# jianzhnie/RLZero

Measured on AMD Instinct MI355X. Metric: mcts_sims_per_sec, higher is better.
Workload: dtype f32 net (hi + lo f16 operand pairs on the f16 MFMA pipe, f32 accumulation) / f64 tree

## Files before the change

### include/rlzero_hip.h

```cpp
#ifndef RLZERO_HIP_H
#define RLZERO_HIP_H

#include <stdint.h>

#ifdef __cplusplus
extern "C" {
#endif

#define RZ_ABI_VERSION 27
#define RZ_MAX_BOARD_SIZE 16
#define RZ_BOARD_WORDS 4
#define RZ_MAX_IN_FLIGHT 16

enum {
    RZ_OK = 0,
    RZ_ERR_ARG = -1,
    RZ_ERR_HIP = -2,
    RZ_ERR_OOM = -3,
    RZ_ERR_OVERFLOW = -4,
    RZ_ERR_ILLEGAL = -5,
    RZ_ERR_INTERNAL = -6
};

enum {
    RZ_GAME_GOMOKU = 0,
    RZ_GAME_CONNECT4 = 1
};

enum {
    RZ_SCORE_UCT_REF = 0,
    RZ_SCORE_PUCT = 1
};

enum { RZ_EVAL_V0 = 0, RZ_EVAL_VLIN = 1 };

enum {
    RZ_FLAG_ARENA_FULL = 1,
    RZ_FLAG_BLOCKS_FULL = 2,
    RZ_FLAG_ILLEGAL_MOVE = 4,
    RZ_FLAG_LOGTAB = 8,
    RZ_FLAG_INTERNAL = 16,
    RZ_FLAG_REUSE_DROPPED = 32
// ... 82 lines not shown
    const float *act_bias;
    const float *val_scale;
    const float *val_bias;
    int64_t raw_part_stride;
    int64_t hid_part_stride;
    int32_t ld;
    int32_t n_parts;
} rz_raw_heads;

int rz_expand_backup_raw(rz_engine *e, const rz_raw_heads *heads, void *stream);
int rz_tree_step_raw(rz_engine *e, const rz_raw_heads *heads, float *d_obs, void *stream);

typedef struct rz_value_head {
    const float *valfeat;
    const float *w1t;
    const float *b1;
    const float *w2;
    const float *b2;
    int32_t ld;
    int32_t groups;
} rz_value_head;
typedef struct rz_deferred_logits {
    const float *raw;
    int32_t ld;
    int32_t rows_per_slot;
} rz_deferred_logits;
int rz_deferred_reserve(rz_engine *e, int32_t slots);
int rz_trace_attach(rz_engine *e, void *d_trace);
int rz_device_view(rz_engine *e, void *out, int64_t out_bytes);
int rz_deferred_slots(rz_engine *e, const int32_t **d_slot_of_game);
int rz_expand_backup_deferred(rz_engine *e, const rz_value_head *head, void *stream);
int rz_tree_step_deferred(rz_engine *e, const rz_value_head *head, void *stream);
int rz_deferred_flush(rz_engine *e, const rz_deferred_logits *logits, int32_t n_slots, void *stream);

int rz_root_visits(rz_engine *e, int32_t *d_visits, void *stream);
int rz_root_wsum(rz_engine *e, double *d_w, void *stream);
int rz_root_priors(rz_engine *e, float *d_p, void *stream);
int rz_root_stats(rz_engine *e, int32_t *d_n, double *d_w, void *stream);
int rz_root_values(rz_engine *e, double *d_out, void *stream);

int rz_advance_roots(rz_engine *e, const int32_t *d_moves, void *stream);

int rz_step_games(rz_engine *e, const int32_t *d_moves, int32_t *d_winner, uint8_t *d_ended,
                  void *stream);

#define RZ_PLAY_RECORD_WORDS 8
enum {
    RZ_PLAY_RUNNING = 1,
    RZ_PLAY_STALLED = 2,
    RZ_PLAY_RESOLVED = 4,
    RZ_PLAY_ENDED = 8,
    RZ_PLAY_SEARCHED = 16,
    RZ_PLAY_RESIGNED = 32,
    RZ_PLAY_NO_RESIGN = 64,
    RZ_PLAY_WOULD_RESIGN = 128
};
typedef struct rz_play_config {
    uint64_t seed;
    double temperature;
    double stall_margin;
    const int64_t *d_queue_ids;
    int32_t *d_queue_ctl;
    int32_t *d_log;
    int32_t ring_steps;
    int32_t reserved;
} rz_play_config;
// ... 16 lines not shown

int rz_uct_scores(rz_engine *e, const double *d_w, const int32_t *d_n, const int32_t *d_np,
                  double c_puct, double *d_out, int64_t count, void *stream);

typedef struct rz_net rz_net;
enum {
    RZ_NET_DIRECT = 0,
    RZ_NET_WINOGRAD_F4 = 1,
    RZ_NET_SPLIT_F16 = 2
    ,
    RZ_NET_SPLIT_F16_TILES = 3
    ,
    RZ_NET_SPLIT_F16_FP8 = 4
};
int rz_net_range_info(rz_net *net, float *h_info8);
enum { RZ_NET_FLAG_F16_RANGE = 1 };
int rz_net_error_flags(rz_net *net, uint32_t *h_flags);
int rz_net_set_algo(rz_net *net, int32_t algo);
int rz_net_set_max_workgroups(rz_net *net, int32_t max_workgroups);
enum { RZ_NET_HEADS_AUTO = 0, RZ_NET_HEADS_F32 = 1, RZ_NET_HEADS_SPLIT_32 = 2, RZ_NET_HEADS_SPLIT_64 = 3, RZ_NET_HEADS_SPLIT_PARTS = 4,
       RZ_NET_HEADS_IN_TRUNK = 5    };
int rz_net_set_heads_algo(rz_net *net, int32_t heads_algo);
int rz_net_create(int32_t height, int32_t width, int32_t n_actions, int32_t device, rz_net **out);
int rz_net_destroy(rz_net *net);
int rz_net_load(rz_net *net, const float *const *h_params, int32_t n_params);
int rz_net_reserve(rz_net *net, int32_t max_boards);
int rz_net_trunk(rz_net *net, const float *d_obs, int32_t n_boards, float *d_feat, void *stream);
int rz_net_trunk_leaves(rz_net *net, const uint64_t *d_stones, const int32_t *d_to_move, const int32_t *d_last_cell,
                        int32_t n_boards, void *stream);
int rz_net_deferred_reserve(rz_net *net, int32_t max_boards, int32_t slots);
int rz_net_trunk_leaves_deferred(rz_net *net, const uint64_t *d_stones, const int32_t *d_to_move, const int32_t *d_last_cell,
                                 int32_t n_boards, const int32_t *d_slot_of_board, rz_value_head *out, void *stream);
int rz_net_deferred_gemm(rz_net *net, int32_t n_boards, int32_t n_slots, rz_deferred_logits *out, void *stream);
int rz_net_trace_attach(rz_net *net, void *d_trace);
int rz_net_delta_reserve(rz_net *net, int32_t n_games);
int rz_net_delta_invalidate(rz_net *net, void *stream);
int rz_net_delta_resident(rz_net *net, int32_t on);
int rz_net_delta_bases(rz_net *net, const uint64_t *d_root_stones, const int32_t *d_root_to_move, int32_t n_games, void *stream);
int rz_net_delta_leaves(rz_net *net, const uint64_t *d_stones, const int32_t *d_to_move, const int32_t *d_last_cell, int32_t n_boards,
                        const int32_t *d_slot_of_board, const uint8_t *d_active, float *d_feat32, int32_t without_base, rz_value_head *out,
                        void *stream);
int rz_net_delta_bases_engine(rz_net *net, rz_engine *engine, void *stream);
int rz_net_delta_step(rz_net *net, rz_engine *engine, rz_value_head *out, void *stream);
int rz_net_delta_trunk_engine(rz_net *net, rz_engine *engine, void *stream);
int rz_net_delta_stats(rz_net *net, uint32_t *h_out8, int32_t reset);
int rz_net_search_resident(rz_net *net, rz_engine *engine, int32_t n_sims, int32_t select_first, void *stream);
int rz_net_heads(rz_net *net, int32_t n_boards, float *d_logp, float *d_value, void *stream);
int rz_net_heads_gemm(rz_net *net, int32_t n_boards, rz_raw_heads *out, void *stream);
int rz_net_forward(rz_net *net, const float *d_obs, int32_t n_boards, float *d_logp,
                   float *d_value, void *stream);

typedef struct rz_muzero rz_muzero;
typedef struct rz_mz_config {
    int32_t abi_version;
    int32_t n_games;
    int32_t n_actions;
    int32_t n_sims;
    double discount;
    double pb_c_base;
    double pb_c_init;
    int32_t device;
    int32_t reserved;
} rz_mz_config;

int rz_mz_create(const rz_mz_config *cfg, rz_muzero **out);
int rz_mz_destroy(rz_muzero *e);
// ... 38 lines not shown
```

### rlzero_amd/_hip.py

```python
import ctypes
import os
from ctypes import (POINTER, Structure, c_char_p, c_double, c_int, c_int32, c_int64, c_uint32, c_uint64,
                    c_void_p)

ABI_VERSION = 27
BOARD_WORDS = 4
MAX_BOARD_SIZE = 16
MAX_IN_FLIGHT = 16

OK = 0
SCORE_UCT_REF, SCORE_PUCT = 0, 1
GAME_GOMOKU, GAME_CONNECT4 = 0, 1
NET_DIRECT, NET_WINOGRAD_F4, NET_SPLIT_F16, NET_SPLIT_F16_TILES, NET_SPLIT_F16_FP8 = 0, 1, 2, 3, 4
NET_FLAG_F16_RANGE = 1
NET_HEADS_AUTO, NET_HEADS_F32, NET_HEADS_SPLIT_32, NET_HEADS_SPLIT_64, NET_HEADS_SPLIT_PARTS, NET_HEADS_IN_TRUNK = 0, 1, 2, 3, 4, 5
EVAL_V0, EVAL_VLIN = 0, 1
FLAG_NAMES = {1: 'arena full', 2: 'block queue full', 4: 'illegal move', 8: 'ln table too short',
              16: 'internal'}
FLAG_REUSE_DROPPED = 32


class RzConfig(Structure):
    _fields_ = [('abi_version', c_int32), ('game_kind', c_int32), ('board_size', c_int32),
                ('n_in_row', c_int32), ('n_games', c_int32), ('n_playout', c_int32),
                ('score_mode', c_int32), ('add_noise', c_int32), ('c_puct', c_double),
                ('pool_factor', c_double), ('device', c_int32), ('noise_seed', c_int32),
                ('board_height', c_int32), ('board_width', c_int32),
                ('sims_in_flight', c_int32), ('in_flight_impl', c_int32)]


class RzStats(Structure):
    _fields_ = [('error_flags', c_int32), ('first_bad_game', c_int32), ('arena_slots', c_int64),
                ('prior_floats', c_int64), ('max_slots_used', c_int64), ('max_blocks_used', c_int64),
                ('device_bytes', c_int64), ('n_select_calls', c_int64), ('reuse_dropped', c_int64)]


class RzMzConfig(Structure):
    _fields_ = [('abi_version', c_int32), ('n_games', c_int32), ('n_actions', c_int32), ('n_sims', c_int32),
# ... 45 lines not shown
    'rz_last_error': (c_char_p, []),
    'rz_source_hash': (c_char_p, []),
    'rz_create': (c_int, [POINTER(RzConfig), POINTER(c_void_p)]),
    'rz_destroy': (c_int, [P]),
    'rz_geometry': (c_int, [P, POINTER(c_int32), POINTER(c_int32), POINTER(c_int32)]),
    'rz_upload_log_table': (c_int, [P, P, c_int64]),
    'rz_log_table_size': (c_int, [P, POINTER(c_int64)]),
    'rz_set_roots': (c_int, [P, P, P, P, P, c_int, P]),
    'rz_get_roots': (c_int, [P, P, P, P, P]),
    'rz_set_active': (c_int, [P, P, P]),
    'rz_set_noise_keys': (c_int, [P, P, P, P]),
    'rz_select_step': (c_int, [P, P, P]),
    'rz_set_in_flight': (c_int, [P, c_int32, c_int32]),
    'rz_leaf_buffers': (c_int, [P, POINTER(c_void_p), POINTER(c_void_p), POINTER(c_void_p)]),
    'rz_encode_leaf_obs': (c_int, [P, P, P]),
    'rz_encode_root_obs': (c_int, [P, P, P]),
    'rz_get_leaves': (c_int, [P, P, P, P, P, P]),
    'rz_eval_synthetic': (c_int, [P, c_int, P, P, P]),
    'rz_eval_rollout': (c_int, [P, c_uint64, c_uint32, c_int32, P, P]),
    'rz_expand_backup': (c_int, [P, P, P, P]),
    'rz_expand_backup_f64': (c_int, [P, P, P, P]),
    'rz_expand_backup_probs': (c_int, [P, P, P, P]),
    'rz_tree_step': (c_int, [P, P, P, P, P]),
    'rz_expand_backup_raw': (c_int, [P, POINTER(RzRawHeads), P]),
    'rz_tree_step_raw': (c_int, [P, POINTER(RzRawHeads), P, P]),
    'rz_trace_attach': (c_int, [P, P]),
    'rz_net_trace_attach': (c_int, [P, P]),
    'rz_device_view': (c_int, [P, P, c_int64]),
    'rz_deferred_reserve': (c_int, [P, c_int32]),
    'rz_deferred_slots': (c_int, [P, POINTER(c_void_p)]),
    'rz_expand_backup_deferred': (c_int, [P, POINTER(RzValueHead), P]),
    'rz_tree_step_deferred': (c_int, [P, POINTER(RzValueHead), P]),
    'rz_deferred_flush': (c_int, [P, POINTER(RzDeferredLogits), c_int32, P]),
    'rz_root_visits': (c_int, [P, P, P]),
    'rz_root_wsum': (c_int, [P, P, P]),
    'rz_root_priors': (c_int, [P, P, P]),
    'rz_root_stats': (c_int, [P, P, P, P]),
    'rz_root_values': (c_int, [P, P, P]),
    'rz_advance_roots': (c_int, [P, P, P]),
    'rz_step_games': (c_int, [P, P, P, P, P]),
    'rz_play_attach': (c_int, [P, POINTER(RzPlayConfig)]),
    'rz_play_draw': (c_int, [P, P]),
    'rz_play_apply': (c_int, [P, P]),
    'rz_play_set_resign': (c_int, [P, c_double, c_double, P]),
    'rz_play_resolve': (c_int, [P, c_int32, c_int32, P]),
    'rz_play_stop': (c_int, [P, P]),
    'rz_play_state': (c_int, [P, P, P, P, POINTER(c_int64)]),
    'rz_get_stats': (c_int, [P, POINTER(RzStats)]),
    'rz_clear_errors': (c_int, [P]),
    'rz_poll_errors': (c_int, [P, POINTER(c_int32), POINTER(c_int32), P]),
    'rz_copy_arena': (c_int, [P, c_int32, c_int64, P, P, P, P, P, P, P, P]),
    'rz_copy_priors': (c_int, [P, c_int32, c_int64, P, P]),
    'rz_uct_scores': (c_int, [P, P, P, P, c_double, P, c_int64, P]),
    'rz_net_create': (c_int, [c_int32, c_int32, c_int32, c_int32, POINTER(c_void_p)]),
    'rz_net_destroy': (c_int, [P]),
    'rz_net_set_algo': (c_int, [P, c_int32]),
    'rz_net_set_max_workgroups': (c_int, [P, c_int32]),
    'rz_net_set_heads_algo': (c_int, [P, c_int32]),
    'rz_net_error_flags': (c_int, [P, POINTER(ctypes.c_uint32)]),
    'rz_net_range_info': (c_int, [P, POINTER(ctypes.c_float)]),
    'rz_net_load': (c_int, [P, POINTER(c_void_p), c_int32]),
    'rz_net_reserve': (c_int, [P, c_int32]),
    'rz_net_trunk': (c_int, [P, P, c_int32, P, P]),
    'rz_net_trunk_leaves': (c_int, [P, P, P, P, c_int32, P]),
    'rz_net_deferred_reserve': (c_int, [P, c_int32, c_int32]),
    'rz_net_trunk_leaves_deferred': (c_int, [P, P, P, P, c_int32, P, POINTER(RzValueHead), P]),
    'rz_net_deferred_gemm': (c_int, [P, c_int32, c_int32, POINTER(RzDeferredLogits), P]),
    'rz_net_search_resident': (c_int, [P, P, c_int32, c_int32, P]),
    'rz_net_delta_reserve': (c_int, [P, c_int32]),
    'rz_net_delta_invalidate': (c_int, [P, P]),
    'rz_net_delta_resident': (c_int, [P, c_int32]),
    'rz_net_delta_bases': (c_int, [P, P, P, c_int32, P]),
    'rz_net_delta_leaves': (c_int, [P, P, P, P, c_int32, P, P, P, c_int32, POINTER(RzValueHead), P]),
    'rz_net_delta_stats': (c_int, [P, POINTER(ctypes.c_uint32), c_int32]),
    'rz_net_delta_bases_engine': (c_int, [P, P, P]),
    'rz_net_delta_step': (c_int, [P, P, POINTER(RzValueHead), P]),
    'rz_net_delta_trunk_engine': (c_int, [P, P, P]),
    'rz_net_heads': (c_int, [P, c_int32, P, P, P]),
    'rz_net_heads_gemm': (c_int, [P, c_int32, POINTER(RzRawHeads), P]),
    'rz_net_forward': (c_int, [P, P, c_int32, P, P, P]),
    'rz_mz_create': (c_int, [POINTER(RzMzConfig), POINTER(c_void_p)]),
    'rz_mz_destroy': (c_int, [P]),
    'rz_mz_upload_log_table': (c_int, [P, P, c_int64]),
    'rz_mz_init_roots': (c_int, [P, P, P, c_double, P, P]),
    'rz_mz_select': (c_int, [P, P, P, P, P, P]),
    'rz_mz_expand_backup': (c_int, [P, P, P, P, P, P]),
    'rz_mz_load_model': (c_int, [P, POINTER(c_void_p), c_int32, c_int32]),
    'rz_mz_search': (c_int, [P, P, c_int32, P, P, P, P, P, P, P]),
    'rz_mz_set_search_shape': (c_int, [P, c_int32]),
    'rz_mz_load_representation': (c_int, [P, POINTER(c_void_p), c_int32, c_int32, c_int32]),
    'rz_mz_play_cartpole': (c_int, [P, P, c_int32, c_int32, POINTER(RzMzCartPolePlay), P]),
    'rz_cartpole_step': (c_int, [P, P, P, P, c_int32, c_uint64, P, P, P, P, P]),
    'rz_mz_root_children': (c_int, [P, c_int32, P, P]),
    'rz_mz_root_stats': (c_int, [P, P, P, P, P, P]),
    'rz_mz_geometry': (c_int, [P, POINTER(c_int32), POINTER(c_int64)]),
    'rz_mz_error_flags': (c_int, [P, POINTER(c_int32)]),
}

_lib = None

# ... 39 lines not shown
```

### rlzero_amd/csrc/rz_engine.hip

```cpp

#include <hip/hip_runtime.h>

#include <cmath>
#include <cstdarg>
#include <cstdio>
#include <cstring>
#include <new>
#include <vector>

#include "rlzero_hip.h"
#include "rz_trace.h"

#pragma clang fp contract(off)

#include "rz_tree.h"

using namespace rzt;

namespace {

__global__ __launch_bounds__(kWave) void k_select(Dev E, float *obs) {
    __builtin_amdgcn_s_setprio(3);
    select_body<false>(E, obs, blockIdx.x, threadIdx.x);
}
// ... 19 lines not shown
template <int PER> constexpr int words_of_per() { return PER <= 4 ? 1 : (PER == 8 ? 2 : kWords); }
template <int PER>
__global__ __launch_bounds__(kWave * kDefWaves) void k_expand_backup_def(Dev E, ValueHead vh) {
    __shared__ float part[kDefWaves][kWave];
    __builtin_amdgcn_s_setprio(3);
    const int lane = threadIdx.x & (kWave - 1), wave = __builtin_amdgcn_readfirstlane(threadIdx.x / kWave);
    value_quarter_def<PER>(vh, blockIdx.x, lane, wave, part);
    if (wave != 0) {
        __syncthreads();
        return;
    }
    expand_backup_body<float, false, false, false, true, words_of_per<PER>()>(E, nullptr, nullptr, blockIdx.x, lane, RawHeads(), 0, vh, part);
}

template <int PER, bool TRACE>
__global__ __launch_bounds__(kWave * kDefWaves) void k_tree_step_def(Dev E, ValueHead vh, float *obs) {
    __shared__ float part[kDefWaves][kWave];
    __builtin_amdgcn_s_setprio(3);
    const int lane = threadIdx.x & (kWave - 1), wave = __builtin_amdgcn_readfirstlane(threadIdx.x / kWave);
    __shared__ unsigned long long trace_t0;
    if (TRACE && threadIdx.x == 0) trace_t0 = rz_trace_now();
    value_quarter_def<PER>(vh, blockIdx.x, lane, wave, part);
    if (wave != 0) {
        __syncthreads();
        return;
    }
    expand_backup_body<float, false, false, false, true, words_of_per<PER>()>(E, nullptr, nullptr, blockIdx.x, lane, RawHeads(), 0, vh, part);
    __syncthreads();
    select_body<false, words_of_per<PER>()>(E, obs, blockIdx.x, lane);
    if (TRACE && lane == 0) rz_trace_write(E.trace, RZ_TRACE_TREE, E.pend[blockIdx.x] - 1, blockIdx.x, trace_t0);
}

__global__ __launch_bounds__(kWave) void k_deferred_priors(Dev E, const float *__restrict__ raw, int ld, long long rows_per_slot) {
    const int g = blockIdx.x, slot = blockIdx.y, lane = threadIdx.x;
    if (slot >= E.pend[g]) return;
    const long long rec = (long long)slot * E.n_games + g;
    const int pb = E.pend_pb[rec];
    if (pb < 0) return;
    const int ctr = E.pend_ctr[rec];
    uint64_t st[2][kWords];
    load_board(E.pend_stones, (int)rec, st);
    const float *r = raw + ((size_t)slot * rows_per_slot + g) * ld;
    float x[kWords];
    float mx = -INFINITY;
#pragma unroll
    for (int i = 0; i < kWords; ++i) {
        const int j = lane + 64 * i;
        x[i] = j < E.A ? r[j] : -INFINITY;
        mx = fmaxf(mx, x[i]);
    }
    mx = wave_max(mx, lane);
    float sum = 0.0f;
#pragma unroll
    for (int i = 0; i < kWords; ++i) sum += (lane + 64 * i < E.A) ? expf(x[i] - mx) : 0.0f;
    sum = wave_sum(sum, lane);
    const float lse = mx + logf(sum);
    float *P = arena_priors(E, g, E.cur_arena[g]);
    uint64_t occ[kWords];
#pragma unroll
    for (int j = 0; j < kWords; ++j) occ[j] = st[0][j] | st[1][j];
    const Legal L = legal_of(E, occ, lane);
    int ranks[kWords];
    int before = 0;
#pragma unroll
    for (int j = 0; j < kWords; ++j) ranks[j] = lane_action_rank(E, occ, L, j, lane, before);
    float noise[kWords] = {0.f, 0.f, 0.f, 0.f};
    float noise_sum = 1.0f;
    if (E.add_noise) {
        const uint64_t key = mix64(mix64(E.noise_key[g]) ^ (uint64_t)ctr);
        float local = 0.0f;
#pragma unroll
        for (int j = 0; j < kWords; ++j)
            if (ranks[j] >= 0) {
                noise[j] = gamma03(hash32((uint32_t)key ^ (uint32_t)(key >> 32)) + 0x9E3779B9u * (uint32_t)(64 * j + lane + 1));
                local += noise[j];
            }
        local = wave_sum(local, lane);
        noise_sum = local > 0.0f ? local : 1.0f;
    }
#pragma unroll
    for (int j = 0; j < kWords; ++j) {
        const int rk = ranks[j];
        if (rk < 0) continue;
        float prior = expf(x[j] - lse);
        if (E.add_noise) prior = 0.75f * prior + 0.25f * (noise[j] / noise_sum);
        P[pb + rk] = prior;
    }
}

__global__ void k_deferred_reset(Dev E) {
    const int g = blockIdx.x * blockDim.x + threadIdx.x;
    if (g < E.n_games) E.pend[g] = 0;
}

template <typename VT>
__global__ __launch_bounds__(kWave) void k_tree_step(Dev E, const float *logp, const VT *value, float *obs) {
    __builtin_amdgcn_s_setprio(3);
    expand_backup_body<VT>(E, logp, value, blockIdx.x, threadIdx.x);
    __syncthreads();
    select_body<false>(E, obs, blockIdx.x, threadIdx.x);
}

template <bool RAW>
__global__ __launch_bounds__(kWave) void k_tree_step_vl(Dev E, const float *logp, const float *value, RawHeads rh,
                                                        float *obs, int kb, int ks) {
    __builtin_amdgcn_s_setprio(3);
#pragma unroll 1
    for (int j = 0; j < kb; ++j) {
        expand_backup_body<float, false, RAW, true>(E, logp, value, blockIdx.x, threadIdx.x, rh, j);
        __syncthreads();
    }
#pragma unroll 1
    for (int j = 0; j < ks; ++j) {
        select_body<true>(E, obs, blockIdx.x, threadIdx.x, j);
        __syncthreads();
    }
}

struct MlSlot {
    uint64_t st[2][kWords];
// ... 1635 lines not shown

int rz_tree_step_deferred(rz_engine *e, const rz_value_head *head, void *stream) {
    int rc = check_engine(e);
    if (rc != RZ_OK) return rc;
    if ((rc = deferred_ok(e, head)) != RZ_OK) return rc;
    e->n_select += 1;
    const dim3 block(kWave * kDefWaves);
    if (e->dev.trace && head->groups == 128) {
        k_tree_step_def<16, true><<<per_game(e), block, 0, as_stream(stream)>>>(e->dev, *head, nullptr);
        return launched("k_tree_step_def");
    }
    switch (head->groups) {
        case 16: k_tree_step_def<2, false><<<per_game(e), block, 0, as_stream(stream)>>>(e->dev, *head, nullptr); break;
        case 32: k_tree_step_def<4, false><<<per_game(e), block, 0, as_stream(stream)>>>(e->dev, *head, nullptr); break;
        case 64: k_tree_step_def<8, false><<<per_game(e), block, 0, as_stream(stream)>>>(e->dev, *head, nullptr); break;
        default: k_tree_step_def<16, false><<<per_game(e), block, 0, as_stream(stream)>>>(e->dev, *head, nullptr); break;
    }
    return launched("k_tree_step_def");
}

int rz_deferred_flush(rz_engine *e, const rz_deferred_logits *logits, int32_t n_slots, void *stream) {
    int rc = check_engine(e);
    if (rc != RZ_OK) return rc;
    if (e->dev.pend_cap <= 0 || n_slots <= 0) return RZ_OK;
    if (!logits || !logits->raw) return fail(RZ_ERR_ARG, "rz_deferred_logits: NULL pointer");
    if (n_slots > e->dev.pend_cap) return fail(RZ_ERR_ARG, "more slots than rz_deferred_reserve()d");
    if (logits->ld < e->dev.A || logits->rows_per_slot < e->cfg.n_games) return fail(RZ_ERR_ARG, "rz_deferred_logits: rows shorter than the batch");
    k_deferred_priors<<<dim3((unsigned)e->cfg.n_games, (unsigned)n_slots), dim3(kWave), 0, as_stream(stream)>>>(
        e->dev, logits->raw, logits->ld, (long long)logits->rows_per_slot);
    if (!(e->play_on && e->play_drawn)) k_deferred_reset<<<flat_grid(e), dim3(256), 0, as_stream(stream)>>>(e->dev);
    return launched("k_deferred_priors");
}

int rz_tree_step_raw(rz_engine *e, const rz_raw_heads *heads, float *d_obs, void *stream) {
    RZ_ENTER(e);
    int rc = raw_heads_ok(e, heads);
    if (rc != RZ_OK) return rc;
    e->n_select += 1;
    const RawHeads rh = *heads;
    if (e->dev.K > 1) {
        if (e->ml) k_tree_step_ml<true><<<per_game(e), dim3(kWave * e->dev.K), e->ml_lds, as_stream(stream)>>>(e->dev, nullptr, nullptr, rh, d_obs, e->kb, e->ks);
        else k_tree_step_vl<true><<<per_game(e), dim3(kWave), 0, as_stream(stream)>>>(e->dev, nullptr, nullptr, rh, d_obs, e->kb, e->ks);
        return launched("k_tree_step_vl");
    }
    k_tree_step_raw<<<per_game(e), dim3(kWave), 0, as_stream(stream)>>>(e->dev, rh, d_obs);
    return launched("k_tree_step_raw");
}

int rz_root_visits(rz_engine *e, int32_t *d_visits, void *stream) {
    RZ_ENTER(e);
    RZ_NEED(d_visits);
    k_root_children<<<per_game(e), dim3(kWave), 0, as_stream(stream)>>>(e->dev, 0, d_visits);
    return launched("k_root_children");
}

int rz_root_wsum(rz_engine *e, double *d_w, void *stream) {
    RZ_ENTER(e);
    RZ_NEED(d_w);
    k_root_children<<<per_game(e), dim3(kWave), 0, as_stream(stream)>>>(e->dev, 1, d_w);
    return launched("k_root_children");
}

int rz_root_priors(rz_engine *e, float *d_p, void *stream) {
    RZ_ENTER(e);
    RZ_NEED(d_p);
    k_root_children<<<per_game(e), dim3(kWave), 0, as_stream(stream)>>>(e->dev, 2, d_p);
// ... 257 lines not shown
```

### rlzero_amd/csrc/rz_net.hip

```cpp

#include <hip/hip_runtime.h>

#include <cmath>
#include <cstdio>
#include <cstring>
#include <new>
#include <type_traits>
#include <utility>
#include <vector>

#include "rlzero_hip.h"
#include "rz_trace.h"
#include "rz_tree.h"
#include "rz_window.h"

void rz_set_error(const char *msg);

namespace {

typedef float f32x4 __attribute__((ext_vector_type(4)));
typedef float f32x2 __attribute__((ext_vector_type(2)));

constexpr int kRowW = 18;
constexpr int kPlaneDirect = 336, kPlaneWino = 337;
// ... 2113 lines not shown
#pragma unroll
            for (int r = 0; r < 16; ++r) dst[(size_t)(8 * (r >> 2) + (r & 3)) * nd.Npad] = fmaf(v[r], scale, bias);
        }
        if (VAL_FUSED) __syncthreads();
    }
    if (vtile >= 0 && vtile < 2) {
        const f32x4 *fb[1] = {nd.fs_val + (size_t)vtile * nd.groups_val * 128};
        sp::f32x16 acc[TM][1];
#pragma unroll
        for (int m = 0; m < TM; ++m)
#pragma unroll
            for (int r = 0; r < 16; ++r) acc[m][0][r] = 0.0f;
        const int K = nd.groups_val, k0 = wave * K / 4, k1 = (wave + 1) * K / 4;
        fs_gemm<TM, 1, DEPTH>(acc, fa, fb, zero, steps_all, nd.groups_act, k0, k1, lane);
#pragma unroll
        for (int m = 0; m < TM; ++m) part[wave][m][lane] = acc[m][0];
        __syncthreads();
        if (wave < TM) {
            const int m = wave;
            sp::f32x16 v = part[0][m][lane];
#pragma unroll
            for (int q = 1; q < 4; ++q) {
                const sp::f32x16 pq = part[q][m][lane];
#pragma unroll
                for (int r = 0; r < 16; ++r) v[r] += pq[r];
            }
            const float scale = nd.s_inv[4];
            const int c = 32 * vtile + col;
            const float bias = nd.fc_val1_b[c];
            float *dst = hid + (size_t)(32 * (mt0 + m) + 4 * h) * 64 + c;
#pragma unroll
            for (int r = 0; r < 16; ++r) dst[(8 * (r >> 2) + (r & 3)) * 64] = fmaxf(fmaf(v[r], scale, bias), 0.0f);
        }
    }
}

template <int DEPTH>
__global__ __launch_bounds__(64) void k_heads_part(NetDev nd, const f32x4 *__restrict__ feat16, float *__restrict__ raw,
                                                   float *__restrict__ hid, long long raw_stride, long long hid_stride) {
    __builtin_amdgcn_s_setprio(3);
    const int lane = threadIdx.x;
    const int mt = blockIdx.x, q = blockIdx.z;
    const int steps_all = nd.groups_act + nd.groups_val;
    const int n_act_tiles = nd.Npad / 32;
    const f32x4 *fa = feat16 + (size_t)mt * steps_all * 128;
    const f32x4 *zero = nd.fs_act + (size_t)n_act_tiles * nd.groups_act * 128;
    const int col = lane & 31, h = lane >> 5;
    const int tile = blockIdx.y;
    const bool is_act = tile < n_act_tiles;
    const int vtile = tile - n_act_tiles;
    const f32x4 *fb[1] = {is_act ? nd.fs_act + (size_t)tile * nd.groups_act * 128 : nd.fs_val + (size_t)vtile * nd.groups_val * 128};
    sp::f32x16 acc[1][1];
#pragma unroll
    for (int r = 0; r < 16; ++r) acc[0][0][r] = 0.0f;
    const int K = is_act ? nd.groups_act : nd.groups_val, k0 = q * K / 4, k1 = (q + 1) * K / 4;
    fs_gemm<1, 1, DEPTH>(acc, fa, fb, zero, steps_all, is_act ? 0 : nd.groups_act, k0, k1, lane);
    float *dst = is_act ? raw + (size_t)q * raw_stride + (size_t)(32 * mt + 4 * h) * nd.Npad + 32 * tile + col
                        : hid + (size_t)q * hid_stride + (size_t)(32 * mt + 4 * h) * 64 + 32 * vtile + col;
    const size_t ld = is_act ? (size_t)nd.Npad : (size_t)64;
#pragma unroll
    for (int r = 0; r < 16; ++r) dst[(size_t)(8 * (r >> 2) + (r & 3)) * ld] = acc[0][0][r];
}

__global__ __launch_bounds__(64) void k_heads_finish(NetDev nd, const float *__restrict__ raw,
                                                     const float *__restrict__ hid, float *__restrict__ logp,
                                                     float *__restrict__ value, int n_boards, int n_parts,
// ... 1026 lines not shown
    if (reset && hipMemset(net->d_delta_stats, 0, 8 * sizeof(uint32_t)) != hipSuccess) return net_fail(RZ_ERR_HIP, "hipMemset failed (delta counters)");
    return RZ_OK;
}

int rz_net_trace_attach(rz_net *net, void *d_trace) {
    if (!net) return net_fail(RZ_ERR_ARG, "net handle is NULL");
    net->d_trace = (unsigned long long *)d_trace;
    return RZ_OK;
}

int rz_net_deferred_gemm(rz_net *net, int32_t n_boards, int32_t n_slots, rz_deferred_logits *out, void *stream) {
    int rc = net_ready(net, n_boards);
    if (rc != RZ_OK) return rc;
    if (!out) return net_fail(RZ_ERR_ARG, "NULL output pointer");
    if (n_slots < 0 || n_slots > net->store_slots || n_boards > net->store_boards)
        return net_fail(RZ_ERR_ARG, "more slots / boards than rz_net_deferred_reserve()d");
    if (n_slots > 0 && n_boards > 0) {
        NetDev nd = net->dev;
        nd.groups_val = 0;
        const int n_act_tiles = nd.Npad / 32, n_groups = (n_act_tiles + 3) / 4;
        if (n_groups > 2) return net_fail(RZ_ERR_INTERNAL, "more than 256 policy outputs");
        const size_t pairs = (size_t)n_slots * net->store_tiles / 2;
        const dim3 grid((unsigned)(n_groups == 2 ? 2 * ((pairs + 7) / 8 * 8) : pairs));
        k_heads_split<2, 4, 3, false, true><<<grid, dim3(256), 0, (hipStream_t)stream>>>(
            nd, reinterpret_cast<const f32x4 *>(net->d_store16), net->d_store_raw, nullptr, n_slots * net->store_tiles * 32);
        if (hipGetLastError() != hipSuccess) return net_fail(RZ_ERR_HIP, "launch of k_heads_split failed");
    }
    out->raw = net->d_store_raw;
    out->ld = net->dev.Npad;
    out->rows_per_slot = net->store_tiles * 32;
    return RZ_OK;
}

int rz_net_set_algo(rz_net *net, int32_t algo) {
    if (!net) return net_fail(RZ_ERR_ARG, "net handle is NULL");
    if (algo != RZ_NET_DIRECT && algo != RZ_NET_WINOGRAD_F4 && algo != RZ_NET_SPLIT_F16 && algo != RZ_NET_SPLIT_F16_TILES &&
        algo != RZ_NET_SPLIT_F16_FP8)
        return net_fail(RZ_ERR_ARG, "unknown algorithm");
    if (algo == RZ_NET_SPLIT_F16_FP8 && !rows_kernel_covers(net->dev.BH, net->dev.BW))
        return net_fail(RZ_ERR_ARG, "RZ_NET_SPLIT_F16_FP8 exists for boards of 11 .. 16 rows and columns (k_trunk_rows)");
    net->fp8_cross = algo == RZ_NET_SPLIT_F16_FP8;
    net->algo = net->fp8_cross ? RZ_NET_SPLIT_F16 : algo;
    return RZ_OK;
}

int rz_net_range_info(rz_net *net, float *h_info8) {
    if (!net || !h_info8) return net_fail(RZ_ERR_ARG, "NULL argument");
    if (!net->loaded) return net_fail(RZ_ERR_ARG, "rz_net_load has not been called");
    memcpy(h_info8, net->range_info, sizeof(net->range_info));
    return RZ_OK;
}

#ifdef RZ_NET_PROFILE
int rz_net_debug_profile(long long *h_out16) {
    return hipDeviceSynchronize() == hipSuccess && hipMemcpyFromSymbol(h_out16, HIP_SYMBOL(net_prof), 24 * sizeof(long long)) == hipSuccess ? RZ_OK : RZ_ERR_HIP;
}
#endif

int rz_net_set_heads_algo(rz_net *net, int32_t heads_algo) {
    if (!net) return net_fail(RZ_ERR_ARG, "net handle is NULL");
    if (heads_algo < RZ_NET_HEADS_AUTO || heads_algo > RZ_NET_HEADS_IN_TRUNK) return net_fail(RZ_ERR_ARG, "unknown heads algorithm");
    net->heads_algo = heads_algo;
    return RZ_OK;
}

int rz_net_set_max_workgroups(rz_net *net, int32_t max_workgroups) {
// ... 57 lines not shown
```

### rlzero_amd/csrc/rz_tree.h

```cpp
#pragma once
#include <hip/hip_runtime.h>

#include <cmath>
#include <stdint.h>

#include "rlzero_hip.h"
#include "rz_trace.h"

#pragma clang fp contract(off)

namespace rzt {
namespace {

constexpr int kWave = 64;
constexpr int kWords = RZ_BOARD_WORDS;

struct Dev {
    int kind, BH, BW, S, A, n_row, n_games, score_mode, n_playout;
    int K;
    int path_stride, qcap;
    long long cap, pcap, logtab_n;
    double c_puct;
    int4 *R;
    float *P;
// ... 948 lines not shown
            a1 = fmaf(fv[i].w, wv[i].w, a1);
        }
        __builtin_amdgcn_sched_barrier(0);
    }
    part[q][lane] = a0 + a1;
}

template <int PER>
__device__ __forceinline__ void value_quarter_lds(const ValueHead &vh, const float *row, int lane, int q, float (*part)[kWave]) {
    typedef float vec4 __attribute__((ext_vector_type(4)));
    const vec4 *w = reinterpret_cast<const vec4 *>(vh.w1t) + (size_t)q * 2 * PER * kWave + lane;
    const vec4 *f = reinterpret_cast<const vec4 *>(row) + q * 2 * PER;
    float a0 = 0.0f, a1 = 0.0f;
#pragma unroll
    for (int half = 0; half < 2; ++half) {
        vec4 wv[PER], fv[PER];
#pragma unroll
        for (int i = 0; i < PER; ++i) {
            wv[i] = w[(size_t)(half * PER + i) * kWave];
            fv[i] = f[half * PER + i];
        }
#pragma unroll
        for (int i = 0; i < PER; ++i) {
            a0 = fmaf(fv[i].x, wv[i].x, a0);
            a1 = fmaf(fv[i].y, wv[i].y, a1);
            a0 = fmaf(fv[i].z, wv[i].z, a0);
            a1 = fmaf(fv[i].w, wv[i].w, a1);
        }
        __builtin_amdgcn_sched_barrier(0);
    }
    part[q][lane] = a0 + a1;
}

}
}
```

### rlzero_amd/engine.py

```python
import ctypes
import functools
import os

import numpy as np

from . import _hip
from . import route as _route
from ._hip import HipError, check
from .route import compact_grid_board

WORDS = _hip.BOARD_WORDS


def _ptr(t):
    return None if t is None else ctypes.c_void_p(t.data_ptr())


_DEVICE_INDEX = {}


def _current_stream(torch, device):
    raw = getattr(torch._C, '_cuda_getCurrentRawStream', None)
    if raw is None:
        return ctypes.c_void_p(torch.cuda.current_stream(device).cuda_stream)
# ... 158 lines not shown

    def delta_bases_engine(self, eng):
        check(self.lib.rz_net_delta_bases_engine(self.handle, eng.handle, self._stream()), 'rz_net_delta_bases_engine')

    def delta_step(self, eng):
        out = _hip.RzValueHead()
        check(self.lib.rz_net_delta_step(self.handle, eng.handle, ctypes.byref(out), self._stream()), 'rz_net_delta_step')
        return out

    def delta_trunk_engine(self, eng):
        check(self.lib.rz_net_delta_trunk_engine(self.handle, eng.handle, self._stream()), 'rz_net_delta_trunk_engine')

    def delta_stats(self, reset=False):
        out = (ctypes.c_uint32 * 8)()
        check(self.lib.rz_net_delta_stats(self.handle, out, 1 if reset else 0), 'rz_net_delta_stats')
        ghz = (256.0 * out[6]) / (10.0 * out[7]) if out[7] else None
        return {'delta': int(out[0]), 'no_base': int(out[1]), 'tiles3': int(out[2]), 'cells': int(out[3]), 'tiles2': int(out[4]),
                'prescans': int(out[5]), 'resident_sclk_ghz': ghz}

    def compact_resident(self):
        return self.route().compact_resident

    def supports_resident(self):
        return self.route(environ={}).resident

    def search_resident(self, eng, n_sims, select_first=False):
        check(self.lib.rz_net_search_resident(self.handle, eng.handle, int(n_sims), 1 if select_first else 0, self._stream()), 'rz_net_search_resident')

    def deferred_gemm(self, n_boards, n_slots):
        out = _hip.RzDeferredLogits()
        check(self.lib.rz_net_deferred_gemm(self.handle, int(n_boards), int(n_slots), ctypes.byref(out), self._stream()),
              'rz_net_deferred_gemm')
        return out

    def range_info(self):
        out = (ctypes.c_float * 8)()
        check(self.lib.rz_net_range_info(self.handle, out), 'rz_net_range_info')
        return {'bounds': (out[0], out[1], out[2]), 'scales': (out[3], out[4], out[5]), 'split_ok': bool(out[6])}

    def check_flags(self):
        flags = ctypes.c_uint32(0)
        check(self.lib.rz_net_error_flags(self.handle, ctypes.byref(flags)), 'rz_net_error_flags')
        if flags.value & _hip.NET_FLAG_F16_RANGE:
            raise HipError("an input outside [0, 1] drove an activation out of the range of the split-f16 trunk: "
                           "use set_algo('direct') for such inputs")
        return self

    def set_heads_algo(self, algo):
        code = {'auto': _hip.NET_HEADS_AUTO, 'f32': _hip.NET_HEADS_F32, 'split32': _hip.NET_HEADS_SPLIT_32,
                'split64': _hip.NET_HEADS_SPLIT_64, 'parts': _hip.NET_HEADS_SPLIT_PARTS, 'in_trunk': _hip.NET_HEADS_IN_TRUNK}[algo]
        check(self.lib.rz_net_set_heads_algo(self.handle, code), 'rz_net_set_heads_algo')
        self.heads_algo = algo
        return self

    def set_max_workgroups(self, n):
        check(self.lib.rz_net_set_max_workgroups(self.handle, int(n)), 'rz_net_set_max_workgroups')
        return self

    def load_state_dict(self, state_dict):
        check_state_dict(state_dict, self.rows, self.cols, self.n_actions)
        arrays = []
        for name in PARAM_ORDER:
            t = state_dict[name]
            a = t.detach().to('cpu', self.torch.float32).contiguous().numpy() if hasattr(t, 'detach') \
                else np.ascontiguousarray(t, dtype=np.float32)
            arrays.append(a)
# ... 533 lines not shown
        return min(n, self._def_slots - self._def_pending)

    def _drop_graphs(self, why):
        if self._graphs or getattr(self, '_move_graph', None) is not None:
            self._graphs = {}
            self._move_graph = None
            self._graphs_dropped = why

    def _sim_chunk_deferred(self, evaluator, n, resident):
        lib, h = self.lib, self.handle
        while n > 0:
            m = self._deferred_begin(evaluator, n)
            if resident:
                evaluator.search_resident(self, m, True)
            else:
                check(lib.rz_select_step(h, None, self.stream()), 'rz_select_step')
                for i in range(m):
                    head = evaluator.deferred_trunk(self)
                    if i + 1 < m:
                        check(lib.rz_tree_step_deferred(h, ctypes.byref(head), self.stream()), 'rz_tree_step_deferred')
                    else:
                        check(lib.rz_expand_backup_deferred(h, ctypes.byref(head), self.stream()), 'rz_expand_backup_deferred')
            if not self._capturing:
                self._def_pending += m
                self._def_stream = self.torch.cuda.current_stream(self.device)
            n -= m

    def flush_deferred(self):
        if self._def_pending <= 0 or self._def_ev is None:
            return
        cur, then = self.torch.cuda.current_stream(self.device), getattr(self, '_def_stream', None)
        if then is not None and then != cur:
            cur.wait_stream(then)
        logits = self._def_ev.hip.deferred_gemm(self.n_leaves, self._def_pending)
        check(self.lib.rz_deferred_flush(self.handle, ctypes.byref(logits), self._def_pending, self.stream()), 'rz_deferred_flush')
        if then is not None and then != cur:
            then.wait_stream(cur)
        self._def_pending = 0

    def _whole_steps(self, n_sims):
        K = self.sims_in_flight
        return max(K, int(n_sims) - int(n_sims) % K)

    def graph_chunk(self, sims_per_graph):
        per = max(1, int(sims_per_graph))
        K = self.sims_in_flight
        if K == 1:
            return per
        full = max(1, self.n_playout // K)
        steps = max(s for s in range(1, min(per, full) + 1) if full % s == 0)
        return K * steps

    def simulate(self, evaluator, n_sims=None, use_graph=False, sims_per_graph=8):
        n = self.n_playout if n_sims is None else int(n_sims)
        r, _, prepare = self._ask(evaluator)
        prepare()
        per = self._whole_steps(sims_per_graph)
        if not use_graph or isinstance(evaluator, HostEvaluator) or r.resident or per > n:
            self.sim_chunk(evaluator, n, r)
            return
        key = (id(evaluator), per)
        if key not in self._graphs:
            why = getattr(self, '_graphs_dropped', None)
            raise HipError('call warm_graph(evaluator, %d) before simulate(use_graph=True)%s' % (per, ' (the graphs were dropped: %s)' % why if why else ''))
        graph = self._graphs[key][0]
        full, rest = divmod(n, per)
        for _ in range(full):
            if r.deferred:
                if self._deferred_begin(evaluator, per) < per:
                    raise HipError('the deferred-priors store (%d slots) is smaller than a graph of %d steps' % (self._def_slots, per))
                self._def_pending += per
# ... 142 lines not shown
        self.active_host[:] = 0
        return self.play_log

    def play_move(self):
        st = self.stream()
        check(self.lib.rz_play_draw(self.handle, st), 'rz_play_draw')
        self.flush_deferred()
        check(self.lib.rz_play_apply(self.handle, st), 'rz_play_apply')
        self.roots_epoch += 1
        row = self.play_steps % self.play_log.shape[0]
        self.play_steps += 1
        return row

    def warm_move_graph(self, evaluator):
        t = self.torch
        r, owner, _ = self._ask(evaluator)
        if not r.resident or getattr(self, 'play_log', None) is None:
            return None
        n = self.n_playout
        self.flush_deferred()
        if self._deferred_begin(evaluator, n) < n or self._def_slots < n:
            return None
        if r.resident_delta:
            owner.reserve_bases(self)
        hip, lib, h = evaluator.hip, self.lib, self.handle
        t.cuda.synchronize(self.device)
        graph = t.cuda.CUDAGraph()
        self._capturing = True
        try:
            with t.cuda.graph(graph):
                st = self.stream()
                evaluator.search_resident(self, n, True)
                check(lib.rz_play_draw(h, st), 'rz_play_draw')
                logits = hip.deferred_gemm(self.n_leaves, n)
                check(lib.rz_deferred_flush(h, ctypes.byref(logits), n, st), 'rz_deferred_flush')
                check(lib.rz_play_apply(h, st), 'rz_play_apply')
        finally:
            self._capturing = False
        self._move_graph_ev = evaluator
        self._move_graph = graph
        self._note_capture(owner or evaluator)
        return graph

    def play_move_replay(self, graph):
        if graph is not getattr(self, '_move_graph', None):
            raise HipError('this whole-move graph was dropped (%s): call warm_move_graph again' % getattr(self, '_graphs_dropped', 'a buffer it addresses moved'))
        if self._def_pending > 0:
            self.flush_deferred()
        graph.replay()
        self.roots_epoch += 1
        row = self.play_steps % self.play_log.shape[0]
        self.play_steps += 1
        return row

    def play_refill(self):
        self.flush_deferred()
        check(self.lib.rz_play_apply(self.handle, self.stream()), 'rz_play_apply')
        self.roots_epoch += 1
        self.play_steps += 1

    def play_set_resign(self, threshold, disabled_frac):
        check(self.lib.rz_play_set_resign(self.handle, float(threshold), float(disabled_frac), self.stream()), 'rz_play_set_resign')
        self.play_resign_on = True

    def play_resolve(self, slot, move):
        check(self.lib.rz_play_resolve(self.handle, int(slot), int(move), self.stream()), 'rz_play_resolve')

    def play_stop(self):
# ... 95 lines not shown
```

Measured before the change: 21.33 million.

## Fuse deferred policy GEMM with prior softmax into a single flush kernel

Adds a fused kernel that computes the deferred policy-head GEMM for a 64-board tile, keeps the logits in shared memory, and then runs the softmax/noise/prior scatter directly from there. The prior body is moved into a shared device function, and a reset entry point is split out. The aim is to avoid the global round-trip for raw logits and one kernel launch per flush. The cost is large shared memory (64 KB per block) and a different GEMM split-K schedule inside the block. The fused path is on by default through an environment switch.

```diff
diff --git a/include/rlzero_hip.h b/include/rlzero_hip.h
--- a/include/rlzero_hip.h
+++ b/include/rlzero_hip.h
@@ -7,7 +7,7 @@
 extern "C" {
 #endif
 
-#define RZ_ABI_VERSION 27
+#define RZ_ABI_VERSION 28
 #define RZ_MAX_BOARD_SIZE 16
 #define RZ_BOARD_WORDS 4
 #define RZ_MAX_IN_FLIGHT 16
@@ -156,6 +156,7 @@
 int rz_expand_backup_deferred(rz_engine *e, const rz_value_head *head, void *stream);
 int rz_tree_step_deferred(rz_engine *e, const rz_value_head *head, void *stream);
 int rz_deferred_flush(rz_engine *e, const rz_deferred_logits *logits, int32_t n_slots, void *stream);
+int rz_deferred_restart(rz_engine *e, void *stream);
 
 int rz_root_visits(rz_engine *e, int32_t *d_visits, void *stream);
 int rz_root_wsum(rz_engine *e, double *d_w, void *stream);
@@ -238,6 +239,7 @@
 int rz_net_trunk_leaves_deferred(rz_net *net, const uint64_t *d_stones, const int32_t *d_to_move, const int32_t *d_last_cell,
                                  int32_t n_boards, const int32_t *d_slot_of_board, rz_value_head *out, void *stream);
 int rz_net_deferred_gemm(rz_net *net, int32_t n_boards, int32_t n_slots, rz_deferred_logits *out, void *stream);
+int rz_net_deferred_flush(rz_net *net, rz_engine *engine, int32_t n_boards, int32_t n_slots, void *stream);
 int rz_net_trace_attach(rz_net *net, void *d_trace);
 int rz_net_delta_reserve(rz_net *net, int32_t n_games);
 int rz_net_delta_invalidate(rz_net *net, void *stream);
diff --git a/rlzero_amd/_hip.py b/rlzero_amd/_hip.py
--- a/rlzero_amd/_hip.py
+++ b/rlzero_amd/_hip.py
@@ -3,7 +3,7 @@
 from ctypes import (POINTER, Structure, c_char_p, c_double, c_int, c_int32, c_int64, c_uint32, c_uint64,
                     c_void_p)
 
-ABI_VERSION = 27
+ABI_VERSION = 28
 BOARD_WORDS = 4
 MAX_BOARD_SIZE = 16
 MAX_IN_FLIGHT = 16
@@ -115,6 +115,7 @@
     'rz_expand_backup_deferred': (c_int, [P, POINTER(RzValueHead), P]),
     'rz_tree_step_deferred': (c_int, [P, POINTER(RzValueHead), P]),
     'rz_deferred_flush': (c_int, [P, POINTER(RzDeferredLogits), c_int32, P]),
+    'rz_deferred_restart': (c_int, [P, P]),
     'rz_root_visits': (c_int, [P, P, P]),
     'rz_root_wsum': (c_int, [P, P, P]),
     'rz_root_priors': (c_int, [P, P, P]),
@@ -149,6 +150,7 @@
     'rz_net_deferred_reserve': (c_int, [P, c_int32, c_int32]),
     'rz_net_trunk_leaves_deferred': (c_int, [P, P, P, P, c_int32, P, POINTER(RzValueHead), P]),
     'rz_net_deferred_gemm': (c_int, [P, c_int32, c_int32, POINTER(RzDeferredLogits), P]),
+    'rz_net_deferred_flush': (c_int, [P, P, c_int32, c_int32, P]),
     'rz_net_search_resident': (c_int, [P, P, c_int32, c_int32, P]),
     'rz_net_delta_reserve': (c_int, [P, c_int32]),
     'rz_net_delta_invalidate': (c_int, [P, P]),
diff --git a/rlzero_amd/csrc/rz_engine.hip b/rlzero_amd/csrc/rz_engine.hip
--- a/rlzero_amd/csrc/rz_engine.hip
+++ b/rlzero_amd/csrc/rz_engine.hip
@@ -75,60 +75,8 @@
 }
 
 __global__ __launch_bounds__(kWave) void k_deferred_priors(Dev E, const float *__restrict__ raw, int ld, long long rows_per_slot) {
-    const int g = blockIdx.x, slot = blockIdx.y, lane = threadIdx.x;
-    if (slot >= E.pend[g]) return;
-    const long long rec = (long long)slot * E.n_games + g;
-    const int pb = E.pend_pb[rec];
-    if (pb < 0) return;
-    const int ctr = E.pend_ctr[rec];
-    uint64_t st[2][kWords];
-    load_board(E.pend_stones, (int)rec, st);
-    const float *r = raw + ((size_t)slot * rows_per_slot + g) * ld;
-    float x[kWords];
-    float mx = -INFINITY;
-#pragma unroll
-    for (int i = 0; i < kWords; ++i) {
-        const int j = lane + 64 * i;
-        x[i] = j < E.A ? r[j] : -INFINITY;
-        mx = fmaxf(mx, x[i]);
-    }
-    mx = wave_max(mx, lane);
-    float sum = 0.0f;
-#pragma unroll
-    for (int i = 0; i < kWords; ++i) sum += (lane + 64 * i < E.A) ? expf(x[i] - mx) : 0.0f;
-    sum = wave_sum(sum, lane);
-    const float lse = mx + logf(sum);
-    float *P = arena_priors(E, g, E.cur_arena[g]);
-    uint64_t occ[kWords];
-#pragma unroll
-    for (int j = 0; j < kWords; ++j) occ[j] = st[0][j] | st[1][j];
-    const Legal L = legal_of(E, occ, lane);
-    int ranks[kWords];
-    int before = 0;
-#pragma unroll
-    for (int j = 0; j < kWords; ++j) ranks[j] = lane_action_rank(E, occ, L, j, lane, before);
-    float noise[kWords] = {0.f, 0.f, 0.f, 0.f};
-    float noise_sum = 1.0f;
-    if (E.add_noise) {
-        const uint64_t key = mix64(mix64(E.noise_key[g]) ^ (uint64_t)ctr);
-        float local = 0.0f;
-#pragma unroll
-        for (int j = 0; j < kWords; ++j)
-            if (ranks[j] >= 0) {
-                noise[j] = gamma03(hash32((uint32_t)key ^ (uint32_t)(key >> 32)) + 0x9E3779B9u * (uint32_t)(64 * j + lane + 1));
-                local += noise[j];
-            }
-        local = wave_sum(local, lane);
-        noise_sum = local > 0.0f ? local : 1.0f;
-    }
-#pragma unroll
-    for (int j = 0; j < kWords; ++j) {
-        const int rk = ranks[j];
-        if (rk < 0) continue;
-        float prior = expf(x[j] - lse);
-        if (E.add_noise) prior = 0.75f * prior + 0.25f * (noise[j] / noise_sum);
-        P[pb + rk] = prior;
-    }
+    const int g = blockIdx.x, slot = blockIdx.y;
+    deferred_priors_body(E, g, slot, threadIdx.x, raw + ((size_t)slot * rows_per_slot + g) * ld);
 }
 
 __global__ void k_deferred_reset(Dev E) {
@@ -1830,6 +1778,14 @@
     return launched("k_deferred_priors");
 }
 
+int rz_deferred_restart(rz_engine *e, void *stream) {
+    int rc = check_engine(e);
+    if (rc != RZ_OK) return rc;
+    if (e->dev.pend_cap <= 0 || (e->play_on && e->play_drawn)) return RZ_OK;
+    k_deferred_reset<<<flat_grid(e), dim3(256), 0, as_stream(stream)>>>(e->dev);
+    return launched("k_deferred_reset");
+}
+
 int rz_tree_step_raw(rz_engine *e, const rz_raw_heads *heads, float *d_obs, void *stream) {
     RZ_ENTER(e);
     int rc = raw_heads_ok(e, heads);
diff --git a/rlzero_amd/csrc/rz_net.hip b/rlzero_amd/csrc/rz_net.hip
--- a/rlzero_amd/csrc/rz_net.hip
+++ b/rlzero_amd/csrc/rz_net.hip
@@ -2169,6 +2169,66 @@
 #pragma unroll
             for (int r = 0; r < 16; ++r) dst[(8 * (r >> 2) + (r & 3)) * 64] = fmaxf(fmaf(v[r], scale, bias), 0.0f);
         }
+    }
+}
+
+constexpr int kFlushDepth = 3;
+__global__ __launch_bounds__(256, 2) void k_flush_fused(NetDev nd, rzt::Dev E, const f32x4 *__restrict__ store16, int store_tiles) {
+    __shared__ float logit[64][256];
+    const int tid = threadIdx.x, lane = tid & 63, wave = __builtin_amdgcn_readfirstlane(tid >> 6);
+    const int mt0 = blockIdx.x * 2;
+    const int slot = mt0 / store_tiles, g0 = (mt0 % store_tiles) * 32;
+    if (g0 >= E.n_games) return;
+    __builtin_amdgcn_s_setprio(3);
+    const int n_act_tiles = nd.Npad / 32, K = nd.groups_act;
+    const f32x4 *fa = store16 + (size_t)mt0 * K * 128;
+    const f32x4 *zero = nd.fs_act + (size_t)n_act_tiles * K * 128;
+    const f32x4 *fb[2];
+#pragma unroll
+    for (int n = 0; n < 2; ++n) fb[n] = 2 * wave + n < n_act_tiles ? nd.fs_act + (size_t)(2 * wave + n) * K * 128 : zero;
+    sp::f32x16 sum[2][2];
+#pragma unroll
+    for (int m = 0; m < 2; ++m)
+#pragma unroll
+        for (int n = 0; n < 2; ++n)
+#pragma unroll
+            for (int r = 0; r < 16; ++r) sum[m][n][r] = 0.0f;
+    fs_gemm<2, 2, kFlushDepth>(sum, fa, fb, zero, K, 0, 0, K / 4, lane);
+#pragma unroll 1
+    for (int q = 1; q < 4; ++q) {
+        sp::f32x16 acc[2][2];
+#pragma unroll
+        for (int m = 0; m < 2; ++m)
+#pragma unroll
+            for (int n = 0; n < 2; ++n)
+#pragma unroll
+                for (int r = 0; r < 16; ++r) acc[m][n][r] = 0.0f;
+        fs_gemm<2, 2, kFlushDepth>(acc, fa, fb, zero, K, 0, q * K / 4, (q + 1) * K / 4, lane);
+#pragma unroll
+        for (int m = 0; m < 2; ++m)
+#pragma unroll
+            for (int n = 0; n < 2; ++n)
+#pragma unroll
+                for (int r = 0; r < 16; ++r) sum[m][n][r] += acc[m][n][r];
+    }
+    const float scale = nd.s_inv[3];
+    const int col = lane & 31, h = lane >> 5;
+#pragma unroll
+    for (int n = 0; n < 2; ++n) {
+        if (2 * wave + n >= n_act_tiles) continue;
+        const int c = 32 * (2 * wave + n) + col;
+        const float bias = nd.fc_act_b[c];
+#pragma unroll
+        for (int m = 0; m < 2; ++m)
+#pragma unroll
+            for (int r = 0; r < 16; ++r) logit[32 * m + 8 * (r >> 2) + 4 * h + (r & 3)][c] = fmaf(sum[m][n][r], scale, bias);
+    }
+    __syncthreads();
+    __builtin_amdgcn_s_setprio(0);
+#pragma unroll 1
+    for (int row = wave; row < 64; row += 4) {
+        const int g = g0 + row;
+        if (g < E.n_games) rzt::deferred_priors_body(E, g, slot, lane, logit[row]);
     }
 }
 
@@ -3261,6 +3321,23 @@
     return RZ_OK;
 }
 
+int rz_net_deferred_flush(rz_net *net, rz_engine *engine, int32_t n_boards, int32_t n_slots, void *stream) {
+    rzt::Dev dev;
+    int rc = rz_device_view(engine, &dev, (int64_t)sizeof(dev));
+    if (rc != RZ_OK) return rc;
+    if ((rc = net_ready(net, n_boards)) != RZ_OK) return rc;
+    if (dev.pend_cap <= 0 || n_slots <= 0) return RZ_OK;
+    if (n_slots > net->store_slots || n_boards > net->store_boards)
+        return net_fail(RZ_ERR_ARG, "more slots / boards than rz_net_deferred_reserve()d");
+    if (n_slots > dev.pend_cap) return net_fail(RZ_ERR_ARG, "more slots than rz_deferred_reserve()d");
+    if (n_boards != dev.n_games || dev.A != net->dev.A) return net_fail(RZ_ERR_ARG, "engine and network disagree on the batch or the board");
+    if (net->dev.Npad > 256) return net_fail(RZ_ERR_INTERNAL, "more than 256 policy outputs");
+    const dim3 grid((unsigned)((size_t)n_slots * net->store_tiles / 2));
+    k_flush_fused<<<grid, dim3(256), 0, (hipStream_t)stream>>>(net->dev, dev, reinterpret_cast<const f32x4 *>(net->d_store16), net->store_tiles);
+    if (hipGetLastError() != hipSuccess) return net_fail(RZ_ERR_HIP, "launch of k_flush_fused failed");
+    return rz_deferred_restart(engine, stream);
+}
+
 int rz_net_set_algo(rz_net *net, int32_t algo) {
     if (!net) return net_fail(RZ_ERR_ARG, "net handle is NULL");
     if (algo != RZ_NET_DIRECT && algo != RZ_NET_WINOGRAD_F4 && algo != RZ_NET_SPLIT_F16 && algo != RZ_NET_SPLIT_F16_TILES &&
diff --git a/rlzero_amd/csrc/rz_tree.h b/rlzero_amd/csrc/rz_tree.h
--- a/rlzero_amd/csrc/rz_tree.h
+++ b/rlzero_amd/csrc/rz_tree.h
@@ -1004,5 +1004,60 @@
     part[q][lane] = a0 + a1;
 }
 
-}
-}
+__device__ __forceinline__ void deferred_priors_body(const Dev &E, int g, int slot, int lane, const float *__restrict__ r) {
+    if (slot >= E.pend[g]) return;
+    const long long rec = (long long)slot * E.n_games + g;
+    const int pb = E.pend_pb[rec];
+    if (pb < 0) return;
+    const int ctr = E.pend_ctr[rec];
+    uint64_t st[2][kWords];
+    load_board(E.pend_stones, (int)rec, st);
+    float x[kWords];
+    float mx = -INFINITY;
+#pragma unroll
+    for (int i = 0; i < kWords; ++i) {
+        const int j = lane + 64 * i;
+        x[i] = j < E.A ? r[j] : -INFINITY;
+        mx = fmaxf(mx, x[i]);
+    }
+    mx = wave_max(mx, lane);
+    float sum = 0.0f;
+#pragma unroll
+    for (int i = 0; i < kWords; ++i) sum += (lane + 64 * i < E.A) ? expf(x[i] - mx) : 0.0f;
+    sum = wave_sum(sum, lane);
+    const float lse = mx + logf(sum);
+    float *P = arena_priors(E, g, E.cur_arena[g]);
+    uint64_t occ[kWords];
+#pragma unroll
+    for (int j = 0; j < kWords; ++j) occ[j] = st[0][j] | st[1][j];
+    const Legal L = legal_of(E, occ, lane);
+    int ranks[kWords];
+    int before = 0;
+#pragma unroll
+    for (int j = 0; j < kWords; ++j) ranks[j] = lane_action_rank(E, occ, L, j, lane, before);
+    float noise[kWords] = {0.f, 0.f, 0.f, 0.f};
+    float noise_sum = 1.0f;
+    if (E.add_noise) {
+        const uint64_t key = mix64(mix64(E.noise_key[g]) ^ (uint64_t)ctr);
+        float local = 0.0f;
+#pragma unroll
+        for (int j = 0; j < kWords; ++j)
+            if (ranks[j] >= 0) {
+                noise[j] = gamma03(hash32((uint32_t)key ^ (uint32_t)(key >> 32)) + 0x9E3779B9u * (uint32_t)(64 * j + lane + 1));
+                local += noise[j];
+            }
+        local = wave_sum(local, lane);
+        noise_sum = local > 0.0f ? local : 1.0f;
+    }
+#pragma unroll
+    for (int j = 0; j < kWords; ++j) {
+        const int rk = ranks[j];
+        if (rk < 0) continue;
+        float prior = expf(x[j] - lse);
+        if (E.add_noise) prior = 0.75f * prior + 0.25f * (noise[j] / noise_sum);
+        P[pb + rk] = prior;
+    }
+}
+
+}
+}
diff --git a/rlzero_amd/engine.py b/rlzero_amd/engine.py
--- a/rlzero_amd/engine.py
+++ b/rlzero_amd/engine.py
@@ -214,6 +214,9 @@
         check(self.lib.rz_net_deferred_gemm(self.handle, int(n_boards), int(n_slots), ctypes.byref(out), self._stream()),
               'rz_net_deferred_gemm')
         return out
+
+    def deferred_flush(self, eng, n_slots, stream):
+        check(self.lib.rz_net_deferred_flush(self.handle, eng.handle, int(eng.n_leaves), int(n_slots), stream), 'rz_net_deferred_flush')
 
     def range_info(self):
         out = (ctypes.c_float * 8)()
@@ -813,11 +816,17 @@
         cur, then = self.torch.cuda.current_stream(self.device), getattr(self, '_def_stream', None)
         if then is not None and then != cur:
             cur.wait_stream(then)
-        logits = self._def_ev.hip.deferred_gemm(self.n_leaves, self._def_pending)
-        check(self.lib.rz_deferred_flush(self.handle, ctypes.byref(logits), self._def_pending, self.stream()), 'rz_deferred_flush')
+        self._flush_launch(self._def_ev.hip, self._def_pending, self.stream())
         if then is not None and then != cur:
             then.wait_stream(cur)
         self._def_pending = 0
+
+    def _flush_launch(self, hip, n_slots, stream):
+        if os.environ.get('RZ_FLUSH_FUSED', '1') != '0':
+            hip.deferred_flush(self, n_slots, stream)
+        else:
+            logits = hip.deferred_gemm(self.n_leaves, n_slots)
+            check(self.lib.rz_deferred_flush(self.handle, ctypes.byref(logits), n_slots, stream), 'rz_deferred_flush')
 
     def _whole_steps(self, n_sims):
         K = self.sims_in_flight
@@ -1026,8 +1035,7 @@
                 st = self.stream()
                 evaluator.search_resident(self, n, True)
                 check(lib.rz_play_draw(h, st), 'rz_play_draw')
-                logits = hip.deferred_gemm(self.n_leaves, n)
-                check(lib.rz_deferred_flush(h, ctypes.byref(logits), n, st), 'rz_deferred_flush')
+                self._flush_launch(hip, n, st)
                 check(lib.rz_play_apply(h, st), 'rz_play_apply')
         finally:
             self._capturing = False
```

Result: no change. 21.26 million (-0.3%).
